# seveirbian/go-libp2p-pubsub

Measured on AMD Instinct MI355X. Metric: peer-message deliveries/sec + gossipsub rounds/sec (node), 1M peers 64 topics, higher is better.
Workload: dtype f64+u64; 1 GPU; config4: 1M peers, 64 topics, k=32, gossipsub v1.1 + Eth2 scoring, 1000 msgs/round, 10 hops/round; peers=1000000, topics=64, degree=32, msgs_per_round=1000, hops_per_round=10, parallelism=replicas1

## Files before the change

go-libp2p-pubsub_amd/csrc/gs_device.h:

```cpp
#pragma once
#include <hip/hip_runtime.h>
#include <stdint.h>

#include "../../include/gossip_engine.h"
#include "../../include/gs_rng.h"
#include "../../include/gs_rpcsize.h"
#include "../../include/gs_trace.h"
#include "../../include/gs_fp.h"

#define GS_WAVE 64
#define GS_WPE_(n) __attribute__((amdgpu_waves_per_eu(n)))
#ifndef GS_WPE_HB
#define GS_WPE_HB 6
#endif
#ifdef GS_WPE_HB
#define GS_OCC_HB GS_WPE_(GS_WPE_HB)
#else
#define GS_OCC_HB
#endif
#ifndef GS_WPE_RF
#define GS_WPE_RF 4
#endif
#ifdef GS_WPE_RF
#define GS_OCC_RF GS_WPE_(GS_WPE_RF)
// ... 434 lines not shown
    if (n == need) {
      sel |= act;
      need = 0;
      break;
    }
  }
  while (need > 0 && act) {
    sel |= act & (~act + 1);
    act &= act - 1;
    need--;
  }
  return (sel >> bl) & 1;
}

__device__ __forceinline__ double add_ones_capped(double x, int n, double cap) {
  return gs_add_ones_capped(x, n, cap);
}

__device__ __forceinline__ int64_t rxi(const Dev& d, int64_t e, int64_t ri) {
  return (ri >= d.e0 && ri < d.e1) ? ri : d.e1 + (e - d.e0);
}
__device__ __forceinline__ uint32_t dlt_get(const Dev& d, int64_t i) {
  if (d.dltN != nullptr) {
    const uint32_t x = d.dltN[i];
    return (x & 0xFFu) | ((x >> 8) << 16);
  }
  return d.dlt[i];
}
__device__ __forceinline__ void dlt_put(const Dev& d, int64_t i, uint32_t q) {
  if (d.dltN != nullptr) d.dltN[i] = (uint16_t)((q & 0xFFu) | ((q >> 16) << 8));
  else d.dlt[i] = q;
}
template <bool NDLT>
__device__ __forceinline__ uint32_t dlt_get_t(const Dev& d, int64_t i) {
  if constexpr (NDLT) {
    const uint32_t x = d.dltN[i];
    return (x & 0xFFu) | ((x >> 8) << 16);
  } else {
    return d.dlt[i];
  }
}
template <bool NDLT>
__device__ __forceinline__ void dlt_put_t(const Dev& d, int64_t i, uint32_t q) {
  if constexpr (NDLT) d.dltN[i] = (uint16_t)((q & 0xFFu) | ((q >> 16) << 8));
  else d.dlt[i] = q;
}
__device__ __forceinline__ double eff_fmd(const TopicP& tp, double fmd, uint32_t q) {
  return (q & 0xFFFF) ? add_ones_capped(fmd, (int)(q & 0xFFFF), tp.FmdCap) : fmd;
}
__device__ __forceinline__ double eff_mmd(const TopicP& tp, double mmd, uint32_t q) {
  return (q >> 16) ? add_ones_capped(mmd, (int)(q >> 16), tp.MmdCap) : mmd;
}

struct TermIn {
  double fmd, mm, mfp, im;
  int64_t mt;
  uint32_t q;
  uint8_t fl;
};
__device__ __forceinline__ int64_t mesh_time_of(int64_t lastRefresh, int64_t gt) {
  return gt <= lastRefresh ? lastRefresh - gt : 0;
}
__device__ __forceinline__ TermIn term_load(const Dev& d, int64_t i) {
  TermIn x;
  x.fl = d.flags[i];
  x.q = dlt_get(d, i);
  x.mt = mesh_time_of(d.lastRefresh, d.graftTime[i]);
  x.mm = d.mmd[i];
  x.fmd = d.fmd[i];
  x.mfp = d.mfp[i];
  x.im = d.anyImd ? d.imd[i] : 0.0;
  return x;
}
__device__ __forceinline__ double term_eval(const TopicP& tp, const TermIn& x) {
  double topicScore = 0.0;
  if (x.fl & 1) {
    double p1 = (double)quantum_div(x.mt, tp);
    if (p1 > tp.TimeInMeshCap) p1 = tp.TimeInMeshCap;
    topicScore += p1 * tp.TimeInMeshWeight;
  }
  topicScore += eff_fmd(tp, x.fmd, x.q) * tp.FmdWeight;
  if (x.fl & 2) {
    const double mm = eff_mmd(tp, x.mm, x.q);
    if (mm < tp.MmdThreshold) {
      const double deficit = tp.MmdThreshold - mm;
      const double p3 = deficit * deficit;
      topicScore += p3 * tp.MmdWeight;
    }
  }
  topicScore += x.mfp * tp.MfpWeight;
  const double p4 = x.im * x.im;
  topicScore += p4 * tp.ImdWeight;
  return topicScore * tp.TopicWeight;
}
__device__ __forceinline__ double topic_term(const Dev& d, const TopicP& tp, int64_t i) {
  return term_eval(tp, term_load(d, i));
}

__device__ __forceinline__ double score_tail_v(const Dev& d, double score, double app, double p6, double b) {
  if (d.TopicScoreCap > 0 && score > d.TopicScoreCap) score = d.TopicScoreCap;
  score += app * d.AppW;
  score += p6 * d.IPW;
  if (b > d.BPThr) {
    const double excess = b - d.BPThr;
    const double p7 = excess * excess;
    score += p7 * d.BPW;
// ... 34 lines not shown
__device__ __forceinline__ void edge_scores_batch(const Dev& d, int64_t rowBase, unsigned long long mask, double& S,
                                                  double* lds) {
  const int lane = lane_id();
  const bool mine = (mask >> lane) & 1;
  if (!d.scoring) {
    if (mine) S = 0.0;
    return;
  }
  const int T = d.T;
  const int tl = lane < T ? lane : 0;
  const bool sc = lane < T && d.tp[tl].scored;
  const uint64_t scoredT = __ballot(sc);
  double app = 0.0, p6 = 0.0, b = 0.0;
  bool rec = false;
  if (mine) {
    const int64_t e = rowBase + lane;
    app = d.app[d.col[e]];
    p6 = d.p6[e];
    b = d.bp[e];
    rec = has_record(d, e);
  }
  while (mask) {
    int js[GS_SBATCH];
#pragma unroll
    for (int k = 0; k < GS_SBATCH; ++k) {
      js[k] = mask ? __ffsll((long long)mask) - 1 : -1;
      mask &= mask ? mask - 1 : 0ull;
    }
    TermIn x[GS_SBATCH];
#pragma unroll
    for (int k = 0; k < GS_SBATCH; ++k) x[k] = term_load(d, tix(d, tl, rowBase + (js[k] < 0 ? js[0] : js[k])));
    __syncthreads();
#pragma unroll
    for (int k = 0; k < GS_SBATCH; ++k) lds[k * 64 + lane] = (js[k] >= 0 && sc) ? term_eval(d.tp[tl], x[k]) : 0.0;
    __syncthreads();
    int kb = -1;
#pragma unroll
    for (int k = 0; k < GS_SBATCH; ++k)
      if (lane == js[k]) kb = k;
    if (kb >= 0) {
      double score = 0.0;
      for (int t = 0; t < T; ++t)
        if ((scoredT >> t) & 1) score += lds[kb * 64 + t];
      S = rec ? score_tail_v(d, score, app, p6, b) : 0.0;
    }
  }
  __syncthreads();
}

__device__ __forceinline__ void stats_graft(const Dev& d, int64_t e, int t, int64_t now) {
  if (!d.scoring || !d.tp[t].scored) return;
  const int64_t i = tix(d, t, e);
  d.sdirty[e] = 1;
  d.flags[i] = 1;
  d.graftTime[i] = now;
  d.meshTime[i] = 0;
}

__device__ __forceinline__ void stats_prune(const Dev& d, int64_t e, int t) {
  if (!d.scoring || !d.tp[t].scored) return;
  const int64_t i = tix(d, t, e);
  d.sdirty[e] = 1;
  const uint8_t fl = d.flags[i];
  const TopicP& tp = d.tp[t];
  const uint32_t q = dlt_get(d, i);
  double mm = d.mmd[i];
  if (q >> 16) {
    mm = eff_mmd(tp, mm, q);
    d.mmd[i] = mm;
    dlt_put(d, i, q & 0xFFFF);
  }
  const double thr = tp.MmdThreshold;
  if ((fl & 2) && mm < thr) {
    const double deficit = thr - mm;
    d.mfp[i] += deficit * deficit;
  }
  if (fl & 1) d.meshTime[i] = mesh_time_of(d.lastRefresh, d.graftTime[i]);
  d.flags[i] = fl & ~1;
}

__device__ __forceinline__ void add_backoff(const Dev& d, int64_t e, int t, int64_t now, int64_t interval) {
  const int64_t i = tix(d, t, e);
  const int64_t expire = now + interval;
  const int64_t cur = d.backoff[i];
  if (cur == 0 || cur < expire) d.backoff[i] = expire;
  d.boMask[e] |= 1ull << t;
}

__device__ __forceinline__ int wave_incl_sum(int x) {
  x += __builtin_amdgcn_update_dpp(0, x, 0x111, 0xF, 0xF, false);
  x += __builtin_amdgcn_update_dpp(0, x, 0x112, 0xF, 0xF, false);
  x += __builtin_amdgcn_update_dpp(0, x, 0x114, 0xF, 0xF, false);
  x += __builtin_amdgcn_update_dpp(0, x, 0x118, 0xF, 0xF, false);
  x += __builtin_amdgcn_update_dpp(0, x, 0x142, 0xA, 0xF, false);
  x += __builtin_amdgcn_update_dpp(0, x, 0x143, 0xC, 0xF, false);
  return x;
}
__device__ __forceinline__ int lane_rank(uint64_t m) {
  return (int)__builtin_amdgcn_mbcnt_hi((unsigned)(m >> 32), __builtin_amdgcn_mbcnt_lo((unsigned)m, 0u));
}
__device__ __forceinline__ bool select_k_lds(bool cand, uint64_t key, int k, uint64_t* skey) {
  (void)skey;
  return select_k(cand, key, k);
}

__device__ __forceinline__ int wave_last(int x) { return __builtin_amdgcn_readlane(x, 63); }

template <int WPL>
__device__ __forceinline__ int64_t arena_write(const Dev& d, int buf, const uint64_t (&bits)[WPL]) {
  const int lane = lane_id();
  int incl[WPL], tot[WPL];
  int total = 0;
#pragma unroll
  for (int j = 0; j < WPL; ++j) {
    const int c = __popcll(bits[j]);
    const int s = wave_incl_sum(c);
    incl[j] = s - c;
    tot[j] = wave_last(s);
    total += tot[j];
  }
  if (total == 0) return -1;
  unsigned long long off = 0;
  if (lane == 0) off = pool_take(d, buf, (unsigned long long)total);
  off = lane_get64(off, 0);
  if (off == ~0ull) return -1;
  int rowBase = (int)off;
#pragma unroll
  for (int j = 0; j < WPL; ++j) {
    int pos = rowBase + incl[j];
    uint64_t y = bits[j];
    while (y) {
// ... 166 lines not shown
```

go-libp2p-pubsub_amd/csrc/gs_engine.hip:

```cpp
#include "gs_engine.h"

static thread_local std::string g_err;
void gs_set_error(const std::string& msg) { g_err = msg; }

static std::vector<int32_t> partition_bounds(const std::vector<int64_t>& rowptr, int N, int world) {
  const int64_t E = rowptr[N];
  std::vector<int32_t> part(world + 1, N);
  part[0] = 0;
  for (int r = 1; r < world; ++r)
    part[r] = (int32_t)(std::lower_bound(rowptr.begin(), rowptr.begin() + N, (E * r) / world) - rowptr.begin());
  for (int r = 1; r <= world; ++r) part[r] = std::max(part[r], part[r - 1]);
  return part;
}

static TopicP to_dev(const gs_topic_score_params& p, bool scored) {
  TopicP t{};
  t.TopicWeight = p.TopicWeight;
  t.TimeInMeshWeight = p.TimeInMeshWeight;
  t.TimeInMeshQuantum = p.TimeInMeshQuantum ? p.TimeInMeshQuantum : 1;
  t.TimeInMeshCap = p.TimeInMeshCap;
  t.FmdWeight = p.FirstMessageDeliveriesWeight;
  t.FmdDecay = p.FirstMessageDeliveriesDecay;
  t.FmdCap = p.FirstMessageDeliveriesCap;
  t.MmdWeight = p.MeshMessageDeliveriesWeight;
// ... 957 lines not shown
          constexpr bool ADV = CV(m) == PA_ADV;
          if constexpr (CV(m) == PA_FLOOD)
            k_flood_a<WV><<<no, 64, 0, stream>>>(d, h, cur, amR, amW, amP);
          else
            k_phase_a<WV, CV(nar), ADV, CV(m) == PA_DENSE>
                <<<no, 64, lds, stream>>>(phaseADev<ADV>(), h, cur, head, amR, amW, amP, amF, nR, nYp);
        }, wpl_of(W), Pick<4>{mode}, Flag{narrow}));
  return GS_OK;
}

int gs_engine::retireAndPublish(const Hop& hp) {
  const int cur = hp.cur, n = hp.n, b = (int)hp.b;
  if (!hp.retireWords.empty()) {
    const int nw = (int)hp.retireWords.size();
    GS_TRY(retireBuf.reserve(hp.retireWords.size()));
    GS_TRY(upload(retireBuf.p, hp.retireWords.data(), hp.retireWords.size() * 4));
    if (nOwn() && (d.spamRow != nullptr || d.pmaskRow != nullptr))
      k_retire<<<nblk((int64_t)nOwn() * nw, 256), 256, 0, stream>>>(d, cur, retireBuf.p, nw);
  }
  if (n > 0) {
    TIMED(this, GS_K_PUBLISH, (k_publish<<<nblk(n, 256), 256, 0, stream>>>(d, b, n, hp.h, cur, head)));
    if (!denseFlood) k_publist<<<nblk(n, 256), 256, 0, stream>>>(d, b, n, cur);
    if (d.sel) k_publish_rs<<<n, 64, 0, stream>>>(d, b);
  }
  return GS_OK;
}

int gs_engine::phaseB(const Hop& hp) {
  const int64_t h = hp.h;
  if (scoring) TIMED(this, GS_K_SCORE, (score_rows<2>(d, eOwn, T, nullptr, stream)));
  int cutMode = 0;
  const int64_t lo = h - (int64_t)(gp.HistoryGossip + 1) * H - maxAge - 2;
  const auto a = std::lower_bound(mHop.begin(), mHop.end(), lo);
  const auto b2 = std::upper_bound(mHop.begin(), mHop.end(), h);
  if ((int64_t)(b2 - a) > (int64_t)gp.MaxIHaveLength) {
    cutMode |= 2;
    std::vector<int64_t> perT((size_t)T, 0);
    for (auto it = a; it != b2; ++it) perT[(size_t)mTopic[(size_t)(it - mHop.begin())]]++;
    for (int t = 0; t < T; ++t)
      if (perT[(size_t)t] > (int64_t)gp.MaxIHaveLength) cutMode |= 1;
  }
  const size_t ldsB = cutMode ? GS_CUTLDS : 0;
  if (cutMode & 1) HIPCHECK(hipMemsetAsync(d.cutSpN, 0, 8, stream));
  if (!nOwn()) return GS_OK;
  GS_TRY(upload(dDev, &d, sizeof(Dev)));
  TIMED(this, GS_K_PHASE_B, with_consts([&](auto w, auto adv) {
          k_phase_b<CV(w) + 1, CV(adv)><<<nOwn(), 64, ldsB, stream>>>(dDev, h, hp.now, hp.cur, head, cutMode);
        }, wpl_of(W), Flag{advModel() || anyPhantom}));
  return GS_OK;
}

void gs_engine::refreshOrFold(const Hop& hp) {
  if (refreshDue(hp.now)) {
    const unsigned rb = nblk(eOwn, GS_RP / T);
    const bool laneT = (64 % T) == 0;
    TIMED(this, GS_K_REFRESH, with_consts([&](auto ndltC, auto churnC, auto laneC) {
            k_refresh_rows<CV(churnC), CV(laneC), CV(ndltC)><<<rb, 64, 0, stream>>>(d, hp.now);
          }, Flag{narrowDlt}, Flag{churnOn}, Flag{laneT}));
    if (churnOn && p6Live() && nOwn()) k_p6<<<nOwn(), 64, 0, stream>>>(d, dP6w);
    refreshedHop = hp.h;
    d.lastRefresh = hp.now;
    hopsSinceFold = 0;
    foldStart = hp.h + 1;
  } else if (scoring && !narrowDlt && ++hopsSinceFold >= foldEvery) {
    k_fold_all<<<nblk(eOwn * T, 256), 256, 0, stream>>>(d);
    hopsSinceFold = 0;
  }
}

void gs_engine::heartbeat(const Hop& hp) {
  const int64_t h = hp.h, now = hp.now;
  const int no = nOwn();
  ticks++;
  if (!directPairs.empty() && ticks % gp.DirectConnectTicks == 0) directConnect();
  const bool exactPass = scoring && (refreshedHop == h || ticks % (uint64_t)d.OGT == 0);
  if (no) TIMED(this, GS_K_HB_PRE, (k_hb_pre<<<no, 64, 0, stream>>>(d, now, ticks, scoring && !exactPass ? 1 : 0)));
  const int allExact = 1;
  if (scoring && refreshedHop == h)
    TIMED(this, GS_K_SCORE, (score_rows<3>(d, eOwn, T, nullptr, stream)));
  else if (scoring && ticks % (uint64_t)d.OGT == 0)
    TIMED(this, GS_K_SCORE, (score_rows<0>(d, eOwn, T, d.score1, stream)));
  else if (scoring)
    TIMED(this, GS_K_SCORE, (score_rows<4>(d, eOwn, T, nullptr, stream)));
  const int newhead = (head + R - 1) % R;
  if (no)
    TIMED(this, GS_K_HEARTBEAT, with_consts([&](auto half) {
            k_heartbeat<CV(half)><<<no, 64, 0, stream>>>(d, h, now, ticks, hp.cur, head, newhead, allExact);
          }, Flag{d.maxDeg <= 32}));
  if (no) {
    k_ptx_rebuild<<<no, 64, (size_t)4 << d.ptxBits, stream>>>(d, (head + d.HL - 1) % R);
    const int64_t nO = (int64_t)1 << d.ptxOBits;
    k_ptxo_collect<<<nblk(nO, 256), 256, 0, stream>>>(d, (head + d.HL - 1) % R);
    k_ptxo_reinsert<<<nblk(nO, 256), 256, 0, stream>>>(d);
    k_ptxo_fin<<<1, 1, 0, stream>>>(d);
  }
  head = newhead;
  heartbeats++;
}

int gs_engine::checkDeviceError() {
  HIPCHECK(hipStreamSynchronize(stream));
  resolveTimings();
  int32_t err = 0;
  HIPCHECK(hipMemcpy(&err, d.err, 4, hipMemcpyDeviceToHost));
  return deviceErrorText(err, -1);
}

// ... 857 lines not shown
    out->gated = (int64_t)c[C_GATED];
  }
  out->hops = g->hop;
  out->heartbeats = g->heartbeats;
  return GS_OK;
}

#define NEED_STARTED(g)                        \
  do {                                         \
    if (!(g)->started) {                       \
      GS_TRY((g)->start());                    \
    }                                          \
  } while (0)

int gs_read_scores(gs_engine* g, double* score) {
  if (!g->graphSet) { gs_set_error("graph not set"); return GS_ESTATE; }
  NEED_STARTED(g);
  score_rows<0>(g->d, g->eOwn, g->d.T, g->dScoreTmp, g->stream);
  std::memset(score, 0, (size_t)g->E * 8);
  HIPCHECK(hipMemcpyAsync(score + g->e0, g->dScoreTmp + g->e0, (size_t)g->eOwn * 8, hipMemcpyDeviceToHost, g->stream));
  HIPCHECK(hipStreamSynchronize(g->stream));
  if (g->mixed)
    for (int u = 0; u < g->N; ++u)
      if (g->routerOf(u) != GS_ROUTER_GOSSIPSUB)
        for (int64_t e = g->rowptr[u]; e < g->rowptr[u + 1]; ++e) score[e] = 0.0;
  return GS_OK;
}

}
template <class X>
static int copy_back_edges(gs_engine* g, X* dst, const X* src) {
  std::memset(dst, 0, (size_t)g->E * sizeof(X));
  if (!g->started) return GS_OK;
  HIPCHECK(hipStreamSynchronize(g->stream));
  HIPCHECK(hipMemcpy(dst + g->e0, src + g->e0, (size_t)g->eOwn * sizeof(X), hipMemcpyDeviceToHost));
  return GS_OK;
}
extern "C" {

int gs_read_mesh(gs_engine* g, uint64_t* mesh) { return copy_back_edges(g, mesh, g->d.mesh); }
int gs_read_fanout(gs_engine* g, uint64_t* fanout) { return copy_back_edges(g, fanout, g->d.fanout); }
int gs_read_backoff(gs_engine* g, int64_t* expire) { return copy_back_pairs(g, expire, g->d.backoff); }
int gs_read_topic_stats(gs_engine* g, double* fmd, double* mmd, double* mfp, double* imd, int64_t* mesh_time,
                        int64_t* graft_time, uint8_t* flags) {
  if (g->started && g->scoring) k_fold_all<<<nblk((int64_t)g->E * g->T, 256), 256, 0, g->stream>>>(g->d);
  GS_TRY(copy_back_pairs(g, fmd, g->d.fmd));
  GS_TRY(copy_back_pairs(g, mmd, g->d.mmd));
  GS_TRY(copy_back_pairs(g, mfp, g->d.mfp));
  GS_TRY(copy_back_pairs(g, imd, g->d.imd));
  GS_TRY(copy_back_pairs(g, mesh_time, (const int64_t*)g->d.meshTime));
  GS_TRY(copy_back_pairs(g, graft_time, (const int64_t*)g->d.graftTime));
  GS_TRY(copy_back_pairs(g, flags, (const uint8_t*)g->d.flags));
  const int64_t lr = g->d.lastRefresh;
  for (int64_t i = 0; i < (int64_t)g->E * g->T; ++i)
    if (flags[i] & 1) mesh_time[i] = graft_time[i] <= lr ? lr - graft_time[i] : 0;
  return GS_OK;
}
int gs_read_behaviour_penalty(gs_engine* g, double* bp) { return copy_back_edges(g, bp, g->d.bp); }

int gs_enough_peers(gs_engine* g, int32_t topic, int32_t suggested, uint8_t* out) {
  if (topic < 0 || topic >= g->T || suggested < 0 || !out) { gs_set_error("gs_enough_peers: bad arguments"); return GS_EINVAL; }
  if (!g->started) { gs_set_error("gs_enough_peers: no state before the first step"); return GS_ESTATE; }
  std::vector<uint64_t> mesh((size_t)g->E);
  GS_TRY(copy_back_edges(g, mesh.data(), g->d.mesh));
  const uint64_t bit = 1ull << topic;
  std::memset(out, 0, (size_t)g->N);
  for (int u = g->n0; u < g->n1; ++u) {
    int fs = 0, rs = 0, gsn = 0, any = 0;
    for (int64_t e = g->rowptr[u]; e < g->rowptr[u + 1]; ++e) {
      if (!g->aliveH.empty() && !g->aliveH[e]) continue;
      if (!(g->subA[g->col[e]] & bit)) continue;
      const int pr = g->protoH[e];
      any++;
      fs += pr == GS_PROTO_FLOODSUB;
      rs += pr == GS_PROTO_RANDOMSUB;
      gsn += (mesh[e] & bit) != 0;
    }
    bool ok;
    switch (g->routerOf(u)) {
      case GS_ROUTER_GOSSIPSUB:
        ok = (fs + rs) + gsn >= (suggested ? suggested : g->gp.Dlo) || gsn >= g->gp.Dhi;
        break;
      case GS_ROUTER_RANDOMSUB:
        ok = fs + rs >= (suggested ? suggested : 6) || rs >= 6;
        break;
      default:
        ok = any >= (suggested ? suggested : 5);
        break;
    }
    out[u] = ok ? 1 : 0;
  }
  return GS_OK;
}

int gs_read_topic_stats_edges(gs_engine* g, int64_t n, const int64_t* edges, double* fmd, double* mmd,
                              double* mfp, double* imd, int64_t* mesh_time, int64_t* graft_time,
                              uint8_t* flags) {
  if (n < 0 || (n > 0 && (!edges || !fmd || !mmd || !mfp || !imd || !mesh_time || !graft_time || !flags))) {
    gs_set_error("gs_read_topic_stats_edges: bad arguments");
    return GS_EINVAL;
  }
  for (int64_t i = 0; i < n; ++i)
    if (edges[i] < 0 || edges[i] >= g->E) { gs_set_error("gs_read_topic_stats_edges: edge out of range"); return GS_EINVAL; }
  const int64_t nk = n * g->T;
  if (!g->started || nk == 0) {
    std::fill(fmd, fmd + nk, 0.0); std::fill(mmd, mmd + nk, 0.0);
    std::fill(mfp, mfp + nk, 0.0); std::fill(imd, imd + nk, 0.0);
    std::fill(mesh_time, mesh_time + nk, 0); std::fill(graft_time, graft_time + nk, 0);
// ... 99 lines not shown
```

go-libp2p-pubsub_amd/csrc/gs_kernels.h:

```cpp
#pragma once
#include <type_traits>

#include "gs_device.h"

#define GS_SB 8
#ifndef GS_RB
#define GS_RB 8
#endif
#define GS_RP 1024
__device__ __forceinline__ int rp_pad(int pl) { return pl + (pl >> 6); }
__host__ __device__ __forceinline__ int score_wave_edges(int T) { return T * 64 <= GS_RP ? 64 : GS_RP / T; }
#define GS_SCW 256
template <int MODE, bool LANE_T>
__global__ __launch_bounds__(64) void k_score_rows(Dev d, double* __restrict__ out) {
  __shared__ double sT[GS_RP + GS_RP / 64];
  __shared__ uint16_t sList[GS_SCW];
  const int lane = lane_id();
  const int T = d.T;
  const int sgw = score_wave_edges(T);
  const int64_t eb = d.e0 + (int64_t)blockIdx.x * GS_SCW;
  int nNeed = 0;
#pragma unroll
  for (int k = 0; k < GS_SCW / 64; ++k) {
    const int64_t e = eb + 64 * k + lane;
    const bool in = e < d.e1;
    double s0 = 0.0;
    bool need = false;
    if (in) {
      if (MODE == 0) {
        need = true;
      } else {
        s0 = d.score0[e];
        need = MODE == 1 ? (d.sdirty[e] != 0 || !(s0 >= d.publishThr))
               : MODE == 2 ? !(s0 >= 0.0)
               : MODE == 4 ? (d.sdirty[e] != 0 || !(s0 >= 0.0))
                           : d.sdirty[e] != 0;
      }
    }
    if (!d.scoring) {
      if (in) {
        if (MODE == 0) out[e] = 0.0;
        if (MODE == 1) { d.score0[e] = 0.0; d.sdirty[e] = 0; }
        if (MODE >= 2) d.score1[e] = 0.0;
      }
      continue;
    }
    if (MODE >= 2 && in && !need) d.score1[e] = s0;
    const unsigned long long m = __ballot(need);
    if (need) sList[nNeed + __popcll(m & ((1ull << lane) - 1))] = (uint16_t)(64 * k + lane);
    nNeed += __popcll(m);
  }
  if (!d.scoring || nNeed == 0) return;
  __syncthreads();
  const int G = LANE_T ? 64 / T : 1;
  const int gi = LANE_T ? lane / T : 0;
  const int tl = LANE_T ? (lane & (T - 1)) : (lane < T ? lane : 0);
  const bool lt = LANE_T || lane < T;
  const bool scoredL = lt && d.tp[tl].scored;
  const uint64_t scoredT = __ballot(lane < T && d.tp[lane < T ? lane : 0].scored);
  for (int c0 = 0; c0 < nNeed; c0 += sgw) {
    const int nc = min(sgw, nNeed - c0);
    const int P = (nc + G - 1) / G;
    for (int p0 = 0; p0 < P; p0 += GS_SB) {
      int js[GS_SB];
#pragma unroll
      for (int k = 0; k < GS_SB; ++k) {
        const int q = (p0 + k) * G + gi;
        js[k] = (lt && q < nc) ? q : -1;
      }
      TermIn x[GS_SB];
#pragma unroll
      for (int k = 0; k < GS_SB; ++k)
        x[k] = term_load(d, (eb + sList[c0 + (js[k] < 0 ? 0 : js[k])]) * T + tl);
#pragma unroll
      for (int k = 0; k < GS_SB; ++k)
        if (js[k] >= 0) sT[rp_pad(js[k] * T + tl)] = scoredL ? term_eval(d.tp[tl], x[k]) : 0.0;
    }
    __syncthreads();
    for (int j = lane; j < nc; j += 64) {
      const int64_t e = eb + sList[c0 + j];
      double score = 0.0;
      for (int t = 0; t < T; ++t)
        if ((scoredT >> t) & 1) score += sT[rp_pad(j * T + t)];
      score = has_record(d, e) ? score_tail(d, e, score) : 0.0;
      if (MODE == 0) out[e] = score;
      if (MODE == 1 || MODE == 3) { d.score0[e] = score; d.sdirty[e] = 0; }
      if (MODE >= 2) d.score1[e] = score;
    }
    __syncthreads();
  }
}

template <bool CHURN, bool LANE_T, bool NDLT>
__global__ __launch_bounds__(64) GS_OCC_RF void k_refresh_rows(Dev d, int64_t now) {
  __shared__ double sT[GS_RP + GS_RP / 64];
  const int lane = lane_id();
  const int T = d.T;
  const int epw = GS_RP / T;
  const int64_t e0 = d.e0 + (int64_t)blockIdx.x * epw;
  const int ng = (int)min((int64_t)epw, d.e1 - e0);
  const int np = ng * T;
  const int64_t p0 = e0 * T;
  const int tl = lane < T ? lane : 0;
  const uint64_t scoredT = __ballot(lane < T && d.tp[tl].scored);
  const int tLane = LANE_T ? (lane & (T - 1)) : 0;
  double tApp = 0.0, tP6 = 0.0, tBp = 0.0;
  if (epw <= 64 && lane < ng) {
    const int64_t e = e0 + lane;
    tApp = d.app[d.col[e]];
    tP6 = d.p6[e];
    tBp = d.bp[e];
  }
  for (int k0 = 0; 64 * k0 < np; k0 += GS_RB) {
    uint32_t q[GS_RB];
    double fmd[GS_RB], mmd[GS_RB], mfp[GS_RB], imd[GS_RB];
    int64_t gt[GS_RB];
    uint8_t fl[GS_RB];
#pragma unroll
    for (int k = 0; k < GS_RB; ++k) {
      const int pl = min(lane + 64 * (k0 + k), np - 1);
      const int64_t i = p0 + pl;
      q[k] = dlt_get_t<NDLT>(d, i);
      fmd[k] = d.fmd[i];
      mmd[k] = d.mmd[i];
      mfp[k] = d.mfp[i];
      imd[k] = d.anyImd ? d.imd[i] : 0.0;
      gt[k] = d.graftTime[i];
      fl[k] = d.flags[i];
    }
#pragma unroll
    for (int k = 0; k < GS_RB; ++k) {
      const int pl = lane + 64 * (k0 + k);
      if (pl >= np) break;
      const int64_t i = p0 + pl;
      int t = tLane;
      int64_t e = 0;
      if (!LANE_T || CHURN) {
        pair_split(d, i, e, t);
        if (LANE_T) t = tLane;
      }
      const TopicP& tp = d.tp[t];
      const bool act = (scoredT >> t) & 1;
      double term = 0.0;
      uint8_t st = 1;
      if (CHURN && d.rstate != nullptr) st = d.rstate[e];
      if (CHURN && st != 1) {
        if (st == 2 && now > d.rexpire[e]) {
          d.fmd[i] = 0; d.mmd[i] = 0; d.mfp[i] = 0; d.imd[i] = 0; dlt_put_t<NDLT>(d, i, 0);
          d.meshTime[i] = 0; d.graftTime[i] = 0; d.flags[i] = 0;
        } else if (act) {
          term = topic_term(d, tp, i);
        }
      } else if (act) {
        TermIn x;
        x.q = 0;
        double v = eff_fmd(tp, fmd[k], q[k]) * tp.FmdDecay;
        if (v < d.DecayToZero) v = 0;
        x.fmd = v;
        v = eff_mmd(tp, mmd[k], q[k]) * tp.MmdDecay;
        if (v < d.DecayToZero) v = 0;
        x.mm = v;
        v = mfp[k] * tp.MfpDecay;
        if (v < d.DecayToZero) v = 0;
        x.mfp = v;
        v = imd[k] * tp.ImdDecay;
        if (v < d.DecayToZero) v = 0;
        x.im = v;
        x.fl = fl[k];
        x.mt = 0;
        if (q[k]) dlt_put_t<NDLT>(d, i, 0);
        if (x.fmd != fmd[k]) d.fmd[i] = x.fmd;
        if (x.mm != mmd[k]) d.mmd[i] = x.mm;
        if (x.mfp != mfp[k]) d.mfp[i] = x.mfp;
        if (d.anyImd && x.im != imd[k]) d.imd[i] = x.im;
        if (x.fl & 1) {
          x.mt = now - gt[k];
          if (x.mt > tp.MmdActivation) {
            x.fl |= 2;
            d.flags[i] = x.fl;
          }
        }
        term = term_eval(tp, x);
      }
      sT[rp_pad(pl)] = term;
    }
  }
  __syncthreads();
  for (int j = lane; j < ng; j += 64) {
    const int64_t e = e0 + j;
    bool frozen = false, dropped = false;
    if (CHURN && d.rstate != nullptr) {
      const uint8_t st = d.rstate[e];
      frozen = st != 1;
      dropped = st == 2 && now > d.rexpire[e];
    }
    const bool pre = epw <= 64;
    double b = pre ? tBp : d.bp[e];
    if (dropped) {
      b = 0;
      d.bp[e] = 0;
      d.rstate[e] = 0;
    } else if (!frozen) {
      b *= d.BPDecay;
      if (b < d.DecayToZero) b = 0;
      d.bp[e] = b;
    }
    double score = 0.0;
    if (d.scoring && !dropped && (!CHURN || has_record(d, e))) {
      for (int t = 0; t < T; ++t)
        if ((scoredT >> t) & 1) score += sT[rp_pad(j * T + t)];
      score = pre ? score_tail_v(d, score, tApp, tP6, b) : score_tail(d, e, score);
    }
    d.score0[e] = score;
    d.sdirty[e] = 0;
  }
}

__global__ void k_fold_all(Dev d) {
  const int64_t p = d.e0 * d.T + (int64_t)blockIdx.x * blockDim.x + threadIdx.x;
  if (p >= d.e1 * d.T) return;
  const uint32_t q = dlt_get(d, p);
  if (!q) return;
  int64_t e;
  int t;
  pair_split(d, p, e, t);
  const TopicP& tp = d.tp[t];
  d.fmd[p] = eff_fmd(tp, d.fmd[p], q);
  d.mmd[p] = eff_mmd(tp, d.mmd[p], q);
  dlt_put(d, p, 0);
}

__global__ void k_gather_pairs(Dev d, const int64_t* __restrict__ edges, int64_t n, uint8_t* __restrict__ out) {
  const int64_t k = (int64_t)blockIdx.x * blockDim.x + threadIdx.x;
  const int64_t nk = n * d.T;
  if (k >= nk) return;
  const int64_t e = edges[k / d.T];
  const int t = (int)(k % d.T);
  double* o = (double*)out;
  int64_t* oi = (int64_t*)out;
  uint8_t* of = out + 48 * nk;
  if (e < d.e0 || e >= d.e1) {
    for (int a = 0; a < 6; ++a) o[a * nk + k] = 0.0;
    of[k] = 0;
    return;
  }
  const int64_t i = tix(d, t, e);
  const TopicP& tp = d.tp[t];
  const uint32_t q = dlt_get(d, i);
  o[k] = eff_fmd(tp, d.fmd[i], q);
  o[nk + k] = eff_mmd(tp, d.mmd[i], q);
  o[2 * nk + k] = d.mfp[i];
  o[3 * nk + k] = d.imd[i];
  oi[4 * nk + k] = (d.flags[i] & 1) ? mesh_time_of(d.lastRefresh, d.graftTime[i]) : d.meshTime[i];
  oi[5 * nk + k] = d.graftTime[i];
  of[k] = d.flags[i];
}

__global__ void k_gather_backoff(Dev d, const int64_t* __restrict__ edges, int64_t n, int64_t* __restrict__ out) {
  const int64_t k = (int64_t)blockIdx.x * blockDim.x + threadIdx.x;
  if (k >= n * d.T) return;
  const int64_t e = edges[k / d.T];
  const int t = (int)(k % d.T);
  out[k] = (e < d.e0 || e >= d.e1) ? 0 : d.backoff[tix(d, t, e)];
}

__global__ void k_fold(Dev d, int t) {
  const int64_t e = d.e0 + (int64_t)blockIdx.x * blockDim.x + threadIdx.x;
  if (e >= d.e1) return;
  const int64_t i = tix(d, t, e);
  const uint32_t q = dlt_get(d, i);
  if (!q) return;
  const TopicP& tp = d.tp[t];
  d.fmd[i] = eff_fmd(tp, d.fmd[i], q);
  d.mmd[i] = eff_mmd(tp, d.mmd[i], q);
  dlt_put(d, i, 0);
}

__global__ void k_recap(Dev d, int t, double fmdCap, double mmdCap) {
  const int64_t e = d.e0 + (int64_t)blockIdx.x * blockDim.x + threadIdx.x;
  if (e >= d.e1) return;
  const int64_t i = tix(d, t, e);
  if (d.fmd[i] > fmdCap) d.fmd[i] = fmdCap;
  if (d.mmd[i] > mmdCap) d.mmd[i] = mmdCap;
}

__global__ __launch_bounds__(64) void k_join(Dev d, int64_t hop, int64_t now, int cur) {
  const int u = d.n0 + blockIdx.x;
  if (!gossip_host(d, u)) return;
  const int lane = lane_id();
  const int64_t base = d.rowptr[u];
  const int deg = (int)(d.rowptr[u + 1] - base);
  const bool valid = lane < deg;
  const int64_t e = base + lane;
  const int v = valid ? d.col[e] : 0;
  const uint64_t subv = valid ? d.subA[v] : 0;
  const bool dir = valid && d.direct[e];
  const double s = valid ? d.score0[e] : 0.0;
  uint64_t meshl = 0, gj = 0;
  const uint64_t joined = d.sub[u];
  for (int t = 0; t < d.T; ++t) {
    if (!((joined >> t) & 1)) continue;
    const bool cand = valid && edge_up(d, e) && mesh_peer(d, e) && ((subv >> t) & 1) && !dir && s >= 0;
    const uint64_t key = gs_key64(d.seed, GS_SITE_GP_JOIN, u, (uint32_t)hop, v, t);
    const bool sel = select_k(cand, key, d.D);
    if (sel) {
      meshl |= 1ull << t;
      gj |= 1ull << t;
      stats_graft(d, e, t, now);
// ... 1825 lines not shown
```

go-libp2p-pubsub_amd/csrc/gs_kernels_ctl.h:

```cpp
#pragma once
#include "gs_device.h"

__device__ __forceinline__ bool graft_one(const Dev& d, int64_t e, int v, int t, double sc, int64_t now,
                                          int& meshcnt_lane, uint64_t& meshE, bool& dirty, bool& dirtyUp,
                                          bool& noPX) {
  if (!((d.sub[v] >> t) & 1)) {
    noPX = true;
    return false;
  }
  if ((meshE >> t) & 1) return false;
  if (d.direct[e]) {
    noPX = true;
    return true;
  }
  const int64_t bi = tix(d, t, e);
  const int64_t be = d.backoff[bi];
  if (be != 0 && now < be) {
    noPX = true;
    if (d.scoring) {
      d.bp[e] += 1.0;
      const int64_t floodCutoff = be + (d.GraftFloodThreshold - d.PruneBackoff);
      if (now < floodCutoff) d.bp[e] += 1.0;
      d.sdirty[e] = 1;
      dirty = true;
// ... 1975 lines not shown
}

__global__ __launch_bounds__(64) void k_edge_down(Dev d, const int32_t* __restrict__ edges, int64_t hop,
                                                  int64_t now, int prv) {
  __shared__ double sterm[64];
  const int64_t e = edges[blockIdx.x];
  const int lane = lane_id();
  const int u = d.esrc[e], v = d.col[e];
  const int64_t re = d.rev[e];
  const bool ownE = e >= d.e0 && e < d.e1;
  const bool ownR = re >= d.e0 && re < d.e1;
  double s = 0.0;
  if (ownE && d.scoring && d.rstate != nullptr && d.rstate[e] == 1) s = edge_score_wave(d, e, sterm);
  if (lane == 0 && ownR) {
    d.cPre[prv][re] = 0; d.cHb[prv][re] = 0; d.cGraftJoin[prv][re] = 0; d.cGraftHb[prv][re] = 0;
    d.cPruneReply[prv][re] = 0; d.cPruneHb[prv][re] = 0; d.cIhave[prv][re] = 0;
    d.cIwant[prv][re] = -1; d.cIresp[prv][re] = -1;
    if (d.cSpam[prv] != nullptr) { d.cSpam[prv][re] = -1; d.cNSrv[prv][re] = 0; }
    if (d.doPX) d.cPx[prv][re] = -1;
    d.fwdIn[prv][re] = make_ulonglong2(0ull, 0ull);
  }
  if (!ownE) return;
  if (lane == 0) {
    d.alive[e] = 0;
    d.mesh[e] = 0;
    d.fanout[e] = 0;
    d.fwdRelay[prv][e] = 0;
    d.fwdPub[prv][e] = 0;
    d.sdirty[e] = 1;
    if (is_traced(d, u)) trace_emit(d, hop, GS_TRACE_REMOVE_PEER, u, v, -1, -1, 0);
    if (d.gater) {
      const int64_t g = d.rowptr[u] + d.gGrp[e];
      atomicSub(&d.gConn[g], 1);
      d.gExp[g] = now + d.gRetain;
    }
  }
  if (!d.scoring || d.rstate == nullptr || d.rstate[e] != 1) return;
  const bool drop = s > 0;
  for (int t = lane; t < d.T; t += 64) {
    const int64_t i = tix(d, t, e);
    if (drop) {
      d.fmd[i] = 0; d.mmd[i] = 0; d.mfp[i] = 0; d.imd[i] = 0; dlt_put(d, i, 0);
      d.meshTime[i] = 0; d.graftTime[i] = 0; d.flags[i] = 0;
      continue;
    }
    if (!d.tp[t].scored) continue;
    const TopicP& tp = d.tp[t];
    const uint32_t q = dlt_get(d, i);
    const double mm = eff_mmd(tp, d.mmd[i], q);
    d.mmd[i] = mm;
    d.fmd[i] = 0;
    dlt_put(d, i, 0);
    const uint8_t fl = d.flags[i];
    if ((fl & 1) && (fl & 2) && mm < tp.MmdThreshold) {
      const double deficit = tp.MmdThreshold - mm;
      d.mfp[i] += deficit * deficit;
    }
    if (fl & 1) d.meshTime[i] = mesh_time_of(d.lastRefresh, d.graftTime[i]);
    d.flags[i] = fl & ~1;
  }
  if (lane == 0) {
    if (drop) {
      d.bp[e] = 0;
      d.rstate[e] = 0;
    } else {
      d.rstate[e] = 2;
      d.rexpire[e] = now + d.RetainScore;
    }
  }
}

__global__ void k_edge_up(Dev d, const int32_t* __restrict__ edges, int n, int64_t hop) {
  const int k = blockIdx.x * blockDim.x + threadIdx.x;
  if (k >= n) return;
  const int64_t e = edges[k];
  if (e < d.e0 || e >= d.e1) return;
  d.alive[e] = 1;
  if (d.rstate != nullptr) d.rstate[e] = 1;
  d.sdirty[e] = 1;
  if (d.gater) atomicAdd(&d.gConn[d.rowptr[d.esrc[e]] + d.gGrp[e]], 1);
  if (is_traced(d, d.esrc[e]))
    trace_emit(d, hop, GS_TRACE_ADD_PEER, d.esrc[e], d.col[e], -1, -1, 0, d.proto ? d.proto[e] : 0);
}

__global__ __launch_bounds__(64) void k_p6(Dev d, double* __restrict__ p6) {
  const int v = d.n0 + blockIdx.x;
  const int lane = lane_id();
  const int64_t base = d.rowptr[v];
  const int deg = (int)(d.rowptr[v + 1] - base);
  const bool valid = lane < deg;
  const int64_t e = base + lane;
  const uint32_t ip = valid ? d.ipv4[d.col[e]] : 0u;
  const bool rec = valid && ip != 0 && has_record(d, e);
  int cnt = 0;
  for (int j = 0; j < deg; ++j) {
    const uint32_t ipj = (uint32_t)__builtin_amdgcn_readlane((int)ip, j);
    const int recj = __builtin_amdgcn_readlane(rec ? 1 : 0, j);
    cnt += (recj && ipj == ip) ? 1 : 0;
  }
  if (!valid) return;
  double f = 0.0;
  if (ip != 0 && !d.ipWL[d.col[e]] && cnt > d.IPThr) {
    const double s = (double)(cnt - d.IPThr);
    f = s * s;
  }
  p6[e] = f;
}

__global__ __launch_bounds__(64) void k_leave(Dev d, const int32_t* __restrict__ items, int64_t hop, int cur) {
  __shared__ double sterm[64];
  const int v = items[3 * blockIdx.x];
  const uint64_t mask = (uint64_t)(uint32_t)items[3 * blockIdx.x + 1] | ((uint64_t)(uint32_t)items[3 * blockIdx.x + 2] << 32);
// ... 153 lines not shown
```

Measured before the change: 4.778 billion deliveries/s.

## Persist refresh blocks over multiple groups with software-pipelined loads and mfp-nonzero flag

k_refresh_rows now handles GS_RG groups of edges per block and prefetches the next turn's inputs while the current ones are being processed. This is meant to hide memory latency and amortise per-block setup, and the per-turn batch GS_RB drops from 8 to 4 to offset the extra registers. A new flag bit records when mfp is nonzero so the refresh can skip loading and decaying mfp for pairs where it is zero. The bit is masked out of the public flags readback. The risks are register pressure and a less parallel grid, and the flag must be maintained at every place that writes mfp.

Result: faster. 5.032 billion deliveries/s (median of 6 runs) (+5.3%).

```diff
diff --git a/go-libp2p-pubsub_amd/csrc/gs_device.h b/go-libp2p-pubsub_amd/csrc/gs_device.h
--- a/go-libp2p-pubsub_amd/csrc/gs_device.h
+++ b/go-libp2p-pubsub_amd/csrc/gs_device.h
@@ -510,6 +510,8 @@
   return (q >> 16) ? add_ones_capped(mmd, (int)(q >> 16), tp.MmdCap) : mmd;
 }
 
+#define GS_FL_MFP 4
+#define GS_FL_PUB 3
 struct TermIn {
   double fmd, mm, mfp, im;
   int64_t mt;
@@ -650,7 +652,7 @@
   if (!d.scoring || !d.tp[t].scored) return;
   const int64_t i = tix(d, t, e);
   d.sdirty[e] = 1;
-  d.flags[i] = 1;
+  d.flags[i] = (d.flags[i] & GS_FL_MFP) | 1;
   d.graftTime[i] = now;
   d.meshTime[i] = 0;
 }
@@ -669,12 +671,14 @@
     dlt_put(d, i, q & 0xFFFF);
   }
   const double thr = tp.MmdThreshold;
+  uint8_t nfl = fl & ~1;
   if ((fl & 2) && mm < thr) {
     const double deficit = thr - mm;
     d.mfp[i] += deficit * deficit;
+    nfl |= GS_FL_MFP;
   }
   if (fl & 1) d.meshTime[i] = mesh_time_of(d.lastRefresh, d.graftTime[i]);
-  d.flags[i] = fl & ~1;
+  d.flags[i] = nfl;
 }
 
 __device__ __forceinline__ void add_backoff(const Dev& d, int64_t e, int t, int64_t now, int64_t interval) {
diff --git a/go-libp2p-pubsub_amd/csrc/gs_engine.hip b/go-libp2p-pubsub_amd/csrc/gs_engine.hip
--- a/go-libp2p-pubsub_amd/csrc/gs_engine.hip
+++ b/go-libp2p-pubsub_amd/csrc/gs_engine.hip
@@ -1033,7 +1033,7 @@
 
 void gs_engine::refreshOrFold(const Hop& hp) {
   if (refreshDue(hp.now)) {
-    const unsigned rb = nblk(eOwn, GS_RP / T);
+    const unsigned rb = nblk(eOwn, GS_RG * (GS_RP / T));
     const bool laneT = (64 % T) == 0;
     TIMED(this, GS_K_REFRESH, with_consts([&](auto ndltC, auto churnC, auto laneC) {
             k_refresh_rows<CV(churnC), CV(laneC), CV(ndltC)><<<rb, 64, 0, stream>>>(d, hp.now);
@@ -1997,8 +1997,10 @@
   GS_TRY(copy_back_pairs(g, graft_time, (const int64_t*)g->d.graftTime));
   GS_TRY(copy_back_pairs(g, flags, (const uint8_t*)g->d.flags));
   const int64_t lr = g->d.lastRefresh;
-  for (int64_t i = 0; i < (int64_t)g->E * g->T; ++i)
+  for (int64_t i = 0; i < (int64_t)g->E * g->T; ++i) {
     if (flags[i] & 1) mesh_time[i] = graft_time[i] <= lr ? lr - graft_time[i] : 0;
+    flags[i] &= GS_FL_PUB;
+  }
   return GS_OK;
 }
 int gs_read_behaviour_penalty(gs_engine* g, double* bp) { return copy_back_edges(g, bp, g->d.bp); }
diff --git a/go-libp2p-pubsub_amd/csrc/gs_kernels.h b/go-libp2p-pubsub_amd/csrc/gs_kernels.h
--- a/go-libp2p-pubsub_amd/csrc/gs_kernels.h
+++ b/go-libp2p-pubsub_amd/csrc/gs_kernels.h
@@ -5,7 +5,7 @@
 
 #define GS_SB 8
 #ifndef GS_RB
-#define GS_RB 8
+#define GS_RB 4
 #endif
 #define GS_RP 1024
 __device__ __forceinline__ int rp_pad(int pl) { return pl + (pl >> 6); }
@@ -56,7 +56,8 @@
   const int gi = LANE_T ? lane / T : 0;
   const int tl = LANE_T ? (lane & (T - 1)) : (lane < T ? lane : 0);
   const bool lt = LANE_T || lane < T;
-  const bool scoredL = lt && d.tp[tl].scored;
+  const TopicP tpL = d.tp[tl];
+  const bool scoredL = lt && tpL.scored;
   const uint64_t scoredT = __ballot(lane < T && d.tp[lane < T ? lane : 0].scored);
   for (int c0 = 0; c0 < nNeed; c0 += sgw) {
     const int nc = min(sgw, nNeed - c0);
@@ -74,7 +75,7 @@
         x[k] = term_load(d, (eb + sList[c0 + (js[k] < 0 ? 0 : js[k])]) * T + tl);
 #pragma unroll
       for (int k = 0; k < GS_SB; ++k)
-        if (js[k] >= 0) sT[rp_pad(js[k] * T + tl)] = scoredL ? term_eval(d.tp[tl], x[k]) : 0.0;
+        if (js[k] >= 0) sT[rp_pad(js[k] * T + tl)] = scoredL ? term_eval(tpL, x[k]) : 0.0;
     }
     __syncthreads();
     for (int j = lane; j < nc; j += 64) {
@@ -91,128 +92,207 @@
   }
 }
 
+#ifndef GS_RG
+#define GS_RG 8
+#endif
+#ifndef GS_RF_TPLDS
+#define GS_RF_TPLDS 0
+#endif
+#ifndef GS_RF_MFPBIT
+#define GS_RF_MFPBIT 1
+#endif
+#define GS_RS (GS_RP / 64)
+constexpr int GS_TPW = (int)(sizeof(TopicP) / 8);
+static_assert(sizeof(TopicP) % 8 == 0, "TopicP is copied to LDS in 64-bit words");
+__device__ __forceinline__ TopicP tp_from_lds(const uint64_t (*s)[64], int t) {
+  uint64_t w[GS_TPW];
+#pragma unroll
+  for (int f = 0; f < GS_TPW; ++f) w[f] = s[f][t];
+  TopicP p;
+  __builtin_memcpy(&p, w, sizeof(TopicP));
+  return p;
+}
+template <class X>
+__device__ __forceinline__ X& at_u(X* base, unsigned c) {
+  return *(X*)((char*)base + (size_t)(c * (unsigned)sizeof(X)));
+}
+struct RfIn {
+  double fmd, mmd, mfp, imd;
+  int64_t gt;
+  uint32_t q;
+  uint16_t qn;
+  uint8_t fl;
+};
 template <bool CHURN, bool LANE_T, bool NDLT>
 __global__ __launch_bounds__(64) GS_OCC_RF void k_refresh_rows(Dev d, int64_t now) {
+  static_assert(GS_RS % GS_RB == 0, "a ring turn stays within one group");
+  constexpr bool TP_REG = LANE_T && !GS_RF_TPLDS;
+  constexpr bool MFPBIT = GS_RF_MFPBIT != 0;
   __shared__ double sT[GS_RP + GS_RP / 64];
+  __shared__ uint64_t sTp[TP_REG ? 1 : GS_TPW][64];
   const int lane = lane_id();
   const int T = d.T;
   const int epw = GS_RP / T;
-  const int64_t e0 = d.e0 + (int64_t)blockIdx.x * epw;
-  const int ng = (int)min((int64_t)epw, d.e1 - e0);
-  const int np = ng * T;
-  const int64_t p0 = e0 * T;
+  const int gPairs = epw * T;
+  const int64_t eW = d.e0 + (int64_t)blockIdx.x * (GS_RG * epw);
+  if (eW >= d.e1) return;
+  const int64_t eEnd = min(d.e1, eW + (int64_t)GS_RG * epw);
+  const int nGrp = (int)((eEnd - eW + epw - 1) / epw);
+  const int64_t pW = eW * T, pEnd = eEnd * T;
   const int tl = lane < T ? lane : 0;
   const uint64_t scoredT = __ballot(lane < T && d.tp[tl].scored);
   const int tLane = LANE_T ? (lane & (T - 1)) : 0;
-  double tApp = 0.0, tP6 = 0.0, tBp = 0.0;
-  if (epw <= 64 && lane < ng) {
-    const int64_t e = e0 + lane;
-    tApp = d.app[d.col[e]];
-    tP6 = d.p6[e];
-    tBp = d.bp[e];
-  }
-  for (int k0 = 0; 64 * k0 < np; k0 += GS_RB) {
-    uint32_t q[GS_RB];
-    double fmd[GS_RB], mmd[GS_RB], mfp[GS_RB], imd[GS_RB];
-    int64_t gt[GS_RB];
-    uint8_t fl[GS_RB];
-#pragma unroll
-    for (int k = 0; k < GS_RB; ++k) {
-      const int pl = min(lane + 64 * (k0 + k), np - 1);
-      const int64_t i = p0 + pl;
-      q[k] = dlt_get_t<NDLT>(d, i);
-      fmd[k] = d.fmd[i];
-      mmd[k] = d.mmd[i];
-      mfp[k] = d.mfp[i];
-      imd[k] = d.anyImd ? d.imd[i] : 0.0;
-      gt[k] = d.graftTime[i];
-      fl[k] = d.flags[i];
-    }
-#pragma unroll
-    for (int k = 0; k < GS_RB; ++k) {
-      const int pl = lane + 64 * (k0 + k);
-      if (pl >= np) break;
-      const int64_t i = p0 + pl;
-      int t = tLane;
-      int64_t e = 0;
-      if (!LANE_T || CHURN) {
-        pair_split(d, i, e, t);
-        if (LANE_T) t = tLane;
-      }
-      const TopicP& tp = d.tp[t];
-      const bool act = (scoredT >> t) & 1;
-      double term = 0.0;
-      uint8_t st = 1;
-      if (CHURN && d.rstate != nullptr) st = d.rstate[e];
-      if (CHURN && st != 1) {
-        if (st == 2 && now > d.rexpire[e]) {
-          d.fmd[i] = 0; d.mmd[i] = 0; d.mfp[i] = 0; d.imd[i] = 0; dlt_put_t<NDLT>(d, i, 0);
-          d.meshTime[i] = 0; d.graftTime[i] = 0; d.flags[i] = 0;
-        } else if (act) {
-          term = topic_term(d, tp, i);
-        }
-      } else if (act) {
-        TermIn x;
-        x.q = 0;
-        double v = eff_fmd(tp, fmd[k], q[k]) * tp.FmdDecay;
-        if (v < d.DecayToZero) v = 0;
-        x.fmd = v;
-        v = eff_mmd(tp, mmd[k], q[k]) * tp.MmdDecay;
-        if (v < d.DecayToZero) v = 0;
-        x.mm = v;
-        v = mfp[k] * tp.MfpDecay;
-        if (v < d.DecayToZero) v = 0;
-        x.mfp = v;
-        v = imd[k] * tp.ImdDecay;
-        if (v < d.DecayToZero) v = 0;
-        x.im = v;
-        x.fl = fl[k];
-        x.mt = 0;
-        if (q[k]) dlt_put_t<NDLT>(d, i, 0);
-        if (x.fmd != fmd[k]) d.fmd[i] = x.fmd;
-        if (x.mm != mmd[k]) d.mmd[i] = x.mm;
-        if (x.mfp != mfp[k]) d.mfp[i] = x.mfp;
-        if (d.anyImd && x.im != imd[k]) d.imd[i] = x.im;
-        if (x.fl & 1) {
-          x.mt = now - gt[k];
-          if (x.mt > tp.MmdActivation) {
-            x.fl |= 2;
-            d.flags[i] = x.fl;
+  TopicP tpR{};
+  if constexpr (TP_REG) {
+    tpR = d.tp[tLane];
+  } else {
+    if (lane < T) {
+      const TopicP g = d.tp[lane];
+      uint64_t w[GS_TPW];
+      __builtin_memcpy(w, &g, sizeof(TopicP));
+#pragma unroll
+      for (int f = 0; f < GS_TPW; ++f) sTp[f][lane] = w[f];
+    }
+    __syncthreads();
+  }
+  auto load = [&](int64_t pB, int rel) -> RfIn {
+    const unsigned c = (unsigned)min(rel + lane, (int)(pEnd - 1 - pB));
+    RfIn x;
+    x.q = 0;
+    x.qn = 0;
+    if constexpr (NDLT) x.qn = at_u(d.dltN + pB, c);
+    else x.q = at_u(d.dlt + pB, c);
+    x.fmd = at_u(d.fmd + pB, c);
+    x.mmd = at_u(d.mmd + pB, c);
+    x.mfp = MFPBIT ? 0.0 : at_u(d.mfp + pB, c);
+    x.imd = d.anyImd ? at_u(d.imd + pB, c) : 0.0;
+    x.gt = at_u(d.graftTime + pB, c);
+    x.fl = at_u(d.flags + pB, c);
+    return x;
+  };
+  const bool pre = epw <= 64;
+  const int64_t eL = min(eW + lane, eEnd - 1);
+  double tP6 = d.p6[eL], tBp = d.bp[eL], tApp = d.app[d.col[eL]];
+  RfIn in[GS_RB];
+#pragma unroll
+  for (int k = 0; k < GS_RB; ++k) in[k] = load(pW, 64 * k);
+  for (int g = 0; g < nGrp; ++g) {
+    const int64_t e0 = eW + (int64_t)g * epw;
+    const int ng = (int)min((int64_t)epw, eEnd - e0);
+    const int np = ng * T;
+    const int64_t p0 = e0 * T;
+    const int64_t eN = min(e0 + epw + lane, eEnd - 1);
+    const uint32_t nCol = (uint32_t)d.col[eN];
+#pragma unroll 1
+    for (int sb = 0; sb < GS_RS; sb += GS_RB) {
+      const bool lastTurn = sb == GS_RS - GS_RB;
+      const int relNext = lastTurn ? gPairs : 64 * (sb + GS_RB);
+#pragma unroll
+      for (int k = 0; k < GS_RB; ++k) {
+        const int pl = 64 * (sb + k) + lane;
+        const unsigned ul = (unsigned)pl;
+        RfIn r = in[k];
+        if constexpr (NDLT) r.q = (r.qn & 0xFFu) | ((uint32_t)(r.qn >> 8) << 16);
+        if (pl < np) {
+          const int64_t i = p0 + pl;
+          int t = tLane;
+          int64_t e = 0;
+          if (!LANE_T || CHURN) {
+            pair_split(d, i, e, t);
+            if (LANE_T) t = tLane;
           }
-        }
-        term = term_eval(tp, x);
-      }
-      sT[rp_pad(pl)] = term;
-    }
-  }
-  __syncthreads();
-  for (int j = lane; j < ng; j += 64) {
-    const int64_t e = e0 + j;
-    bool frozen = false, dropped = false;
-    if (CHURN && d.rstate != nullptr) {
-      const uint8_t st = d.rstate[e];
-      frozen = st != 1;
-      dropped = st == 2 && now > d.rexpire[e];
-    }
-    const bool pre = epw <= 64;
-    double b = pre ? tBp : d.bp[e];
-    if (dropped) {
-      b = 0;
-      d.bp[e] = 0;
-      d.rstate[e] = 0;
-    } else if (!frozen) {
-      b *= d.BPDecay;
-      if (b < d.DecayToZero) b = 0;
-      d.bp[e] = b;
-    }
-    double score = 0.0;
-    if (d.scoring && !dropped && (!CHURN || has_record(d, e))) {
-      for (int t = 0; t < T; ++t)
-        if ((scoredT >> t) & 1) score += sT[rp_pad(j * T + t)];
-      score = pre ? score_tail_v(d, score, tApp, tP6, b) : score_tail(d, e, score);
-    }
-    d.score0[e] = score;
-    d.sdirty[e] = 0;
+          if constexpr (LANE_T && !TP_REG) asm volatile("" : "+v"(t));
+          const TopicP tp = TP_REG ? tpR : tp_from_lds(sTp, t);
+          const bool act = (scoredT >> t) & 1;
+          double term = 0.0;
+          uint8_t st = 1;
+          if (CHURN && d.rstate != nullptr) st = d.rstate[e];
+          if (CHURN && st != 1) {
+            if (st == 2 && now > d.rexpire[e]) {
+              d.fmd[i] = 0; d.mmd[i] = 0; d.mfp[i] = 0; d.imd[i] = 0; dlt_put_t<NDLT>(d, i, 0);
+              d.meshTime[i] = 0; d.graftTime[i] = 0; d.flags[i] = 0;
+            } else if (act) {
+              term = topic_term(d, tp, i);
+            }
+          } else if (act) {
+            TermIn x;
+            x.q = 0;
+            double v = eff_fmd(tp, r.fmd, r.q) * tp.FmdDecay;
+            if (v < d.DecayToZero) v = 0;
+            x.fmd = v;
+            v = eff_mmd(tp, r.mmd, r.q) * tp.MmdDecay;
+            if (v < d.DecayToZero) v = 0;
+            x.mm = v;
+            x.fl = r.fl;
+            x.mfp = 0.0;
+            if (!MFPBIT || (r.fl & GS_FL_MFP)) {
+              const double m = MFPBIT ? at_u(d.mfp + p0, ul) : r.mfp;
+              v = m * tp.MfpDecay;
+              if (v < d.DecayToZero) v = 0;
+              if (v != m) at_u(d.mfp + p0, ul) = v;
+              if (v == 0) x.fl &= ~GS_FL_MFP;
+              x.mfp = v;
+            }
+            v = r.imd * tp.ImdDecay;
+            if (v < d.DecayToZero) v = 0;
+            x.im = v;
+            x.mt = 0;
+            if (r.q) {
+              if constexpr (NDLT) at_u(d.dltN + p0, ul) = 0;
+              else at_u(d.dlt + p0, ul) = 0;
+            }
+            if (x.fmd != r.fmd) at_u(d.fmd + p0, ul) = x.fmd;
+            if (x.mm != r.mmd) at_u(d.mmd + p0, ul) = x.mm;
+            if (d.anyImd && x.im != r.imd) at_u(d.imd + p0, ul) = x.im;
+            if (x.fl & 1) {
+              x.mt = now - r.gt;
+              if (x.mt > tp.MmdActivation) x.fl |= 2;
+            }
+            if (x.fl != r.fl) at_u(d.flags + p0, ul) = x.fl;
+            term = term_eval(tp, x);
+          }
+          sT[rp_pad(pl)] = term;
+        }
+        in[k] = load(p0, relNext + 64 * k);
+      }
+    }
+    __syncthreads();
+    auto sums = [&](auto preC) {
+    constexpr bool pre = decltype(preC)::value;
+    for (int j = lane; j < ng; j += 64) {
+      const int64_t e = e0 + j;
+      bool frozen = false, dropped = false;
+      if (CHURN && d.rstate != nullptr) {
+        const uint8_t st = d.rstate[e];
+        frozen = st != 1;
+        dropped = st == 2 && now > d.rexpire[e];
+      }
+      double b = pre ? tBp : d.bp[e];
+      if (dropped) {
+        b = 0;
+        d.bp[e] = 0;
+        d.rstate[e] = 0;
+      } else if (!frozen) {
+        b *= d.BPDecay;
+        if (b < d.DecayToZero) b = 0;
+        d.bp[e] = b;
+      }
+      double score = 0.0;
+      if (d.scoring && !dropped && (!CHURN || has_record(d, e))) {
+        for (int t = 0; t < T; ++t)
+          if ((scoredT >> t) & 1) score += sT[rp_pad(j * T + t)];
+        score = pre ? score_tail_v(d, score, tApp, tP6, b) : score_tail(d, e, score);
+      }
+      d.score0[e] = score;
+      d.sdirty[e] = 0;
+    }
+    };
+    if (pre) sums(std::true_type{});
+    else sums(std::false_type{});
+    __syncthreads();
+    tP6 = d.p6[eN];
+    tBp = d.bp[eN];
+    tApp = d.app[nCol];
   }
 }
 
@@ -253,7 +333,7 @@
   o[3 * nk + k] = d.imd[i];
   oi[4 * nk + k] = (d.flags[i] & 1) ? mesh_time_of(d.lastRefresh, d.graftTime[i]) : d.meshTime[i];
   oi[5 * nk + k] = d.graftTime[i];
-  of[k] = d.flags[i];
+  of[k] = d.flags[i] & GS_FL_PUB;
 }
 
 __global__ void k_gather_backoff(Dev d, const int64_t* __restrict__ edges, int64_t n, int64_t* __restrict__ out) {
diff --git a/go-libp2p-pubsub_amd/csrc/gs_kernels_ctl.h b/go-libp2p-pubsub_amd/csrc/gs_kernels_ctl.h
--- a/go-libp2p-pubsub_amd/csrc/gs_kernels_ctl.h
+++ b/go-libp2p-pubsub_amd/csrc/gs_kernels_ctl.h
@@ -2051,12 +2051,14 @@
     d.fmd[i] = 0;
     dlt_put(d, i, 0);
     const uint8_t fl = d.flags[i];
+    uint8_t nfl = fl & ~1;
     if ((fl & 1) && (fl & 2) && mm < tp.MmdThreshold) {
       const double deficit = tp.MmdThreshold - mm;
       d.mfp[i] += deficit * deficit;
+      nfl |= GS_FL_MFP;
     }
     if (fl & 1) d.meshTime[i] = mesh_time_of(d.lastRefresh, d.graftTime[i]);
-    d.flags[i] = fl & ~1;
+    d.flags[i] = nfl;
   }
   if (lane == 0) {
     if (drop) {
```
